# simonsobs/pixell

Measured on AMD Instinct MI355X. Metric: map2alm+alm2map round-trips/sec, higher is better.
Workload: dtype f64

## Files before the change

pixell_amd/csrc/leg_s0.hip:

```cpp
#include "legendre_dev.hpp"

namespace pxs {

#define S0_PHASE_A \
	while (k + 4 <= nk) { \
		bool act = false; \
		_Pragma("unroll") for (int s = 0; s < K; s++) act |= LEG_IS_LIVE(lam2[s], sc[s]); \
		if (__any(act)) break; \
		const double4_t q0 = LDC(coef, k), q1 = LDC(coef, k+1), q2 = LDC(coef, k+2), q3 = LDC(coef, k+3); \
		const double b0 = polar ? q0.c : q0.b, b1 = polar ? q1.c : q1.b, b2 = polar ? q2.c : q2.b, b3 = polar ? q3.c : q3.b; \
		_Pragma("unroll") for (int s = 0; s < K; s++) { \
			lam1[s] = fma(fma(q0.a, csq[s], b0), lam2[s], lam1[s]); \
			lam2[s] = fma(fma(q1.a, csq[s], b1), lam1[s], lam2[s]); \
			lam1[s] = fma(fma(q2.a, csq[s], b2), lam2[s], lam1[s]); \
			lam2[s] = fma(fma(q3.a, csq[s], b3), lam1[s], lam2[s]); \
			if (sc[s] < 0 && fabs(lam2[s]) > SC_BIG) { lam1[s] *= SC_SMALL; lam2[s] *= SC_SMALL; sc[s]++; } \
		} \
		k += 4; \
	}
#define S0_SEEDED_PHASE_A \
	if (a.seed_mode == 2) { \
		const double* sd = a.seed_d + ((long)m*a.nwave + wv)*(2*K*64); const int* si = a.seed_i + ((long)m*a.nwave + wv)*((K+1)*64); \
		k = PXS_UNIFORM_INT(si[K*64]); \
		_Pragma("unroll") for (int s = 0; s < K; s++) { lam1[s] = sd[s*64 + lane]; lam2[s] = sd[(K+s)*64 + lane]; sc[s] = si[s*64 + lane]; } \
// ... 117 lines not shown
	double t0 = 0, t1 = 0, t2 = 0, t3 = 0, u0 = 0, u1 = 0, u2 = 0, u3 = 0; \
	_Pragma("unroll") for (int s = 0; s < K; s++) { \
		t0 = fma(lam2[s], d1r[s], t0); t1 = fma(lam2[s], d1i[s], t1); t2 = fma(lam2[s], d2r[s], t2); t3 = fma(lam2[s], d2i[s], t3); \
		lam1[s] = fma(fma(c0.a, csq[s], vb0), lam2[s], lam1[s]); \
	} \
	_Pragma("unroll") for (int s = 0; s < K; s++) { \
		u0 = fma(lam1[s], d1r[s], u0); u1 = fma(lam1[s], d1i[s], u1); u2 = fma(lam1[s], d2r[s], u2); u3 = fma(lam1[s], d2i[s], u3); \
		lam2[s] = fma(fma(c1.a, csq[s], vb1), lam1[s], lam2[s]); \
	} \
	 \
	LEG_RED_PUT(kk, t0, t1, t2, t3) \
	LEG_RED_PUT(kk+1, u0, u1, u2, u3) \
	kk += 2; \
	if (kk == LEG_FSTEPS) { leg_flush(red, pout + 4*kbase, lane, LEG_FSTEPS, a.atomic); kk = 0; kbase = k+2; } }

template<int K> __global__ __launch_bounds__(64) void leg_ana_s0(const LegK a)
{
	PXS_SHARED(double, red);
	const int lane = threadIdx.x; int wv, m, bb;
	if (!leg_block(a, wv, m, bb)) return;
	const long row0 = PXS_UNIFORM_LONG(a.row[m]);
	const int nk = (a.lmax - m)/2 + 1;
	const double4_t* __restrict__ coef = a.coef + row0;
	double* __restrict__ pout = a.part + (long)bb*a.mom_bs + ((long)wv*a.rows_chunk + (row0 - a.rowbase))*4;
	const double2* __restrict__ in = a.leg + (long)bb*a.leg_bs + (long)m*a.ld;
	double csq[K], lam1[K], lam2[K], d1r[K], d1i[K], d2r[K], d2i[K];
	int sc[K];
	bool alive_any = false;
	const bool polar = leg_wave_polar(a, wv, K);
	auto load_data = [&](int s) {
		const int p = leg_pair(a, wv, K, s, lane);
		const bool valid = leg_pair_valid(a, p);
		const int rn = valid ? a.ring_n[p] : -1, rs = valid ? a.ring_s[p] : -1;
		const double x = valid ? a.cth[p] : 0.0;
		const double2 vn = rn >= 0 ? in[rn] : make_double2(0, 0);
		const double2 vs = rs >= 0 ? in[rs] : make_double2(0, 0);
		d1r[s] = vn.x + vs.x; d1i[s] = vn.y + vs.y;
		d2r[s] = (vn.x - vs.x)*x; d2i[s] = (vn.y - vs.y)*x;
	};
#pragma unroll
	for (int s = 0; s < K; s++) {
		const int p = leg_pair(a, wv, K, s, lane);
		const bool valid = leg_pair_valid(a, p);
		const double x = valid ? a.cth[p] : 0.0;
		const double sth = valid ? a.sth[p] : 0.0;
		csq[s] = polar ? -sth*sth : x*x;
// ... 16 lines not shown
		bool pend = false;
#pragma unroll
		for (int s = 0; s < K; s++) pend |= (sc[s] < 0);
		if (!__any(pend)) break;
		for (int it = 0; it < 2 && k + 1 < nk; it++, k += 2) {
			const double4_t c0 = LDC(coef, k), c1 = LDC(coef, k+1);
			S0_ANA_PAIR(c0, c1)
		}
#pragma unroll
		for (int s = 0; s < K; s++)
			if (sc[s] < 0 && fabs(lam2[s]) > SC_BIG) {
				lam1[s] *= SC_SMALL; lam2[s] *= SC_SMALL;
				if (++sc[s] == 0) load_data(s);
			}
	}
	double4_t c0 = LDC(coef, k), c1 = LDC(coef, k+1);
	while (k + 3 < nk) {
		double4_t n0 = LDC(coef, k+2), n1 = LDC(coef, k+3);
		S0_ANA_PAIR(c0, c1)
		k += 2;
		c0 = LDC(coef, k+2); c1 = LDC(coef, k+3);
		S0_ANA_PAIR(n0, n1)
		k += 2;
	}
	for (; k + 1 < nk; k += 2) {
		const double4_t n0 = LDC(coef, k+2), n1 = LDC(coef, k+3);
		S0_ANA_PAIR(c0, c1)
		c0 = n0; c1 = n1;
	}
	if (k < nk) {
		double t0 = 0, t1 = 0, t2 = 0, t3 = 0;
#pragma unroll
		for (int s = 0; s < K; s++) { t0 = fma(lam2[s], d1r[s], t0); t1 = fma(lam2[s], d1i[s], t1); t2 = fma(lam2[s], d2r[s], t2); t3 = fma(lam2[s], d2i[s], t3); }
		LEG_RED_PUT(kk, t0, t1, t2, t3)
		kk++;
	}
	if (kk > 0) leg_flush(red, pout + 4*kbase, lane, kk, a.atomic);
}


struct S0Chain {
	double csq, lam1, lam2; int sc;
	__device__ __forceinline__ double step(double ca, double cb) { const double p = lam2, nx = fma(mm_coef(ca, csq, cb), lam2, lam1); lam1 = p; lam2 = nx; return p; }
	__device__ __forceinline__ void rescale() { if (fabs(lam2) > SC_BIG) { lam1 *= SC_SMALL; lam2 *= SC_SMALL; sc++; } }
// ... 65 lines not shown
					const double val = c < 2 ? fma(x, o, v) : fma(-x, v, o);
					const int ring = valid ? (c < 2 ? a.ring_n[p] : a.ring_s[p]) : -1;
					if (ring >= 0) out[2*ring] = val;
				}
		}
	}
};
template<int NG, int W> __global__ __launch_bounds__(64*W, 4) void leg_ana_s0_mm(const LegK a) { leg_ana_mm<S0Mm, NG, W>(a); }



template<int NG> __global__ __launch_bounds__(64, 4) void leg_syn_s0_mm(const LegK a) { leg_syn_mm<S0Mm, NG>(a); }

void launch_leg_s0(bool analysis, int ng, int K, dim3 grid, hipStream_t st, const LegK& a) {
	static const bool once = leg_mm_lds_optin({leg_ana_s0_mm<2, MM_WAVES>, leg_ana_s0_mm<1, MM_WAVES>}); (void)once;
	const LegKernel k = analysis ? (ng == 2 ? leg_ana_s0_mm<2, MM_WAVES> : ng ? leg_ana_s0_mm<1, MM_WAVES> : K == 8 ? leg_ana_s0<8> : K == 2 ? leg_ana_s0<2> : leg_ana_s0<4>)
	                             : (ng == 2 ? leg_syn_s0_mm<2> : ng ? leg_syn_s0_mm<1> : K == 2 ? leg_syn_s0<2> : leg_syn_s0<4>);
	leg_launch(k, analysis, ng, grid, st, a);
}

}
```

pixell_amd/csrc/leg_spin.hip:

```cpp
#include "legendre_dev.hpp"

namespace pxs {

template<int K> struct SpinState {
	double x[K], gp1[K], gp2[K], gm1[K], gm2[K];
	int scp[K], scm[K];
};

template<int K> __device__ __forceinline__ bool spin_init(const LegK& a, int wv, int lane, int m, SpinState<K>& S, int* rn, int* rs, bool polar) {
	const int s_ = a.spin;
	bool alive_any = false;
#pragma unroll
	for (int s = 0; s < K; s++) {
		const int p = leg_pair(a, wv, K, s, lane);
		const bool valid = leg_pair_valid(a, p);
		rn[s] = valid ? a.ring_n[p] : -1; rs[s] = valid ? a.ring_s[p] : -1;
		const double cth = valid ? a.cth[p] : 0.0;
		const double sth = valid ? a.sth[p] : 0.0;
		const double shh = valid ? a.sh2[p] : 0.0;
		S.x[s] = polar ? -2.0*shh*shh : cth;
		const double t1 = a.lmax*sth + a.ofs;
		const double b = -2.0*s_*fabs(cth);
		const double c = (double)s_*s_ - t1*t1;
		const double discr = b*b - 4*c;
// ... 45 lines not shown
		j = PXS_UNIFORM_INT(si[2*K*64]); \
		_Pragma("unroll") for (int s = 0; s < K; s++) { \
			S.gp1[s] = sd[s*64 + lane]; S.gp2[s] = sd[(K+s)*64 + lane]; S.gm1[s] = sd[(2*K+s)*64 + lane]; S.gm2[s] = sd[(3*K+s)*64 + lane]; \
			S.scp[s] = si[s*64 + lane]; S.scm[s] = si[(K+s)*64 + lane]; } \
	} else { \
		SPIN_PHASE_A \
		if (a.seed_mode == 1) { \
			double* sd = a.seed_d + ((long)m*a.nwave + wv)*(4*K*64); int* si = a.seed_i + ((long)m*a.nwave + wv)*((2*K+1)*64); \
			_Pragma("unroll") for (int s = 0; s < K; s++) { \
				sd[s*64 + lane] = S.gp1[s]; sd[(K+s)*64 + lane] = S.gp2[s]; sd[(2*K+s)*64 + lane] = S.gm1[s]; sd[(3*K+s)*64 + lane] = S.gm2[s]; \
				si[s*64 + lane] = S.scp[s]; si[(K+s)*64 + lane] = S.scm[s]; } \
			if (lane == 0) si[2*K*64] = j; \
		} \
	}

#define SPIN_SYN_PAIR(f0, f1, a0, a1) { \
	{ \
		const double ca = f0.a, c1 = polar ? f0.c : f0.b, c2 = polar ? f0.d : -f0.b; \
		PXS_VCOPY(v1, c1); PXS_VCOPY(v2, c2); \
		_Pragma("unroll") for (int s = 0; s < K; s++) { \
			const double gp = S.gp2[s], gm = S.gm2[s]; \
			pnr[s] = fma(gp, a0.a, pnr[s]); pni[s] = fma(gp, a0.b, pni[s]); \
			mnr[s] = fma(gm, a0.c, mnr[s]); mni[s] = fma(gm, a0.d, mni[s]); \
			qsr[s] = fma(gm, a0.a, qsr[s]); qsi[s] = fma(gm, a0.b, qsi[s]); \
			nsr[s] = fma(gp, a0.c, nsr[s]); nsi[s] = fma(gp, a0.d, nsi[s]); \
			S.gp1[s] = fma(fma(ca, S.x[s], v1), gp, -S.gp1[s]); S.gm1[s] = fma(fma(ca, S.x[s], v2), gm, -S.gm1[s]); \
		} \
	} \
	{ \
		const double ca = f1.a, c1 = polar ? f1.c : f1.b, c2 = polar ? f1.d : -f1.b; \
		PXS_VCOPY(v1, c1); PXS_VCOPY(v2, c2); \
		_Pragma("unroll") for (int s = 0; s < K; s++) { \
			const double gp = S.gp1[s], gm = S.gm1[s]; \
			pnr[s] = fma(gp, a1.a, pnr[s]); pni[s] = fma(gp, a1.b, pni[s]); \
			mnr[s] = fma(gm, a1.c, mnr[s]); mni[s] = fma(gm, a1.d, mni[s]); \
			qsr[s] = fma(-gm, a1.a, qsr[s]); qsi[s] = fma(-gm, a1.b, qsi[s]); \
			nsr[s] = fma(-gp, a1.c, nsr[s]); nsi[s] = fma(-gp, a1.d, nsi[s]); \
			S.gp2[s] = fma(fma(ca, S.x[s], v1), gp, -S.gp2[s]); S.gm2[s] = fma(fma(ca, S.x[s], v2), gm, -S.gm2[s]); \
		} \
	} }

template<int K> __global__ __launch_bounds__(64) void leg_syn_spin(const LegK a)
{
	const int lane = threadIdx.x; int wv, m, bb;
	if (!leg_block(a, wv, m, bb)) return;
	const int l0 = max(m, a.spin);
	const int nl = a.lmax - l0 + 1;
	double2* __restrict__ outq = a.leg + (long)bb*a.leg_bs + (long)m*a.ld;
	double2* __restrict__ outu = a.leg + (long)bb*a.leg_bs + ((long)a.nm + m)*a.ld;
	SpinState<K> S; int rn[K], rs[K];
	double pnr[K], pni[K], mnr[K], mni[K], qsr[K], qsi[K], nsr[K], nsi[K];
#pragma unroll
	for (int s = 0; s < K; s++) pnr[s] = pni[s] = mnr[s] = mni[s] = qsr[s] = qsi[s] = nsr[s] = nsi[s] = 0;
	const bool polar = leg_wave_polar(a, wv, K);
	const bool alive_any = spin_init<K>(a, wv, lane, m, S, rn, rs, polar);
// ... 18 lines not shown
			}
#pragma unroll
			for (int s = 0; s < K; s++) {
				const bool was = (S.scp[s] < 0) || (S.scm[s] < 0);
				if (S.scp[s] < 0 && fabs(S.gp2[s]) > SC_BIG) { S.gp1[s] *= SC_SMALL; S.gp2[s] *= SC_SMALL; S.scp[s]++; }
				if (S.scm[s] < 0 && fabs(S.gm2[s]) > SC_BIG) { S.gm1[s] *= SC_SMALL; S.gm2[s] *= SC_SMALL; S.scm[s]++; }
				if (was && S.scp[s] == 0 && S.scm[s] == 0) pnr[s] = pni[s] = mnr[s] = mni[s] = qsr[s] = qsi[s] = nsr[s] = nsi[s] = 0;
			}
		}
#pragma unroll
		for (int s = 0; s < K; s++)
			if (S.scp[s] < 0 || S.scm[s] < 0) {
				pnr[s] = pni[s] = mnr[s] = mni[s] = qsr[s] = qsi[s] = nsr[s] = nsi[s] = 0;
				S.gp1[s] = S.gp2[s] = S.gm1[s] = S.gm2[s] = 0;
			}
		double4_t f0 = LDC(coef, j), f1 = LDC(coef, j+1), a0 = LDC(at, j), a1 = LDC(at, j+1);
		while (j + 3 < nl) {
			double4_t n0 = LDC(coef, j+2), n1 = LDC(coef, j+3), m0 = LDC(at, j+2), m1 = LDC(at, j+3);
			SPIN_SYN_PAIR(f0, f1, a0, a1)
			j += 2;
			f0 = LDC(coef, j+2); f1 = LDC(coef, j+3); a0 = LDC(at, j+2); a1 = LDC(at, j+3);
			SPIN_SYN_PAIR(n0, n1, m0, m1)
			j += 2;
		}
		for (; j + 1 < nl; j += 2) {
			const double4_t n0 = LDC(coef, j+2), n1 = LDC(coef, j+3), m0 = LDC(at, j+2), m1 = LDC(at, j+3);
			SPIN_SYN_PAIR(f0, f1, a0, a1)
			f0 = n0; f1 = n1; a0 = m0; a1 = m1;
		}
		if (j < nl) {
#pragma unroll
			for (int s = 0; s < K; s++) {
				const double gp = S.gp2[s], gm = S.gm2[s];
				pnr[s] = fma(gp, a0.a, pnr[s]); pni[s] = fma(gp, a0.b, pni[s]);
				mnr[s] = fma(gm, a0.c, mnr[s]); mni[s] = fma(gm, a0.d, mni[s]);
				qsr[s] = fma(gm, a0.a, qsr[s]); qsi[s] = fma(gm, a0.b, qsi[s]);
				nsr[s] = fma(gp, a0.c, nsr[s]); nsi[s] = fma(gp, a0.d, nsi[s]);
			}
		}
	}
#pragma unroll
	for (int s = 0; s < K; s++) {
		const int p = leg_pair(a, wv, K, s, lane);
		const bool valid = leg_pair_valid(a, p);
// ... 30 lines not shown
		_Pragma("unroll") for (int s = 0; s < K; s++) { \
			const double gp = S.gp1[s], gm = S.gm1[s]; \
			u0 = fma(gp, tpnr[s], u0); u0 = fma(-gm, tpsr[s], u0); \
			u1 = fma(gp, tpni[s], u1); u1 = fma(-gm, tpsi[s], u1); \
			u2 = fma(gm, tmnr[s], u2); u2 = fma(-gp, tmsr[s], u2); \
			u3 = fma(gm, tmni[s], u3); u3 = fma(-gp, tmsi[s], u3); \
			S.gp2[s] = fma(fma(ca, S.x[s], v1), gp, -S.gp2[s]); S.gm2[s] = fma(fma(ca, S.x[s], v2), gm, -S.gm2[s]); \
		} \
	} \
	 \
	LEG_RED_PUT(kk, t0, t1, t2, t3) \
	LEG_RED_PUT(kk+1, u0, u1, u2, u3) \
	kk += 2; \
	if (kk == LEG_FSTEPS) { leg_flush(red, pout + 4*jbase, lane, LEG_FSTEPS, a.atomic); kk = 0; jbase = j+2; } }

template<int K> __global__ __launch_bounds__(64) void leg_ana_spin(const LegK a)
{
	PXS_SHARED(double, red);
	const int lane = threadIdx.x; int wv, m, bb;
	if (!leg_block(a, wv, m, bb)) return;
	const int l0 = max(m, a.spin);
	const int nl = a.lmax - l0 + 1;
	if (nl <= 0) return;
	const long row0 = PXS_UNIFORM_LONG(a.row[m]);
	const double4_t* __restrict__ coef = a.coef + row0;
	double* __restrict__ pout = a.part + (long)bb*a.mom_bs + ((long)wv*a.rows_chunk + (row0 - a.rowbase))*4;
	const double2* __restrict__ inq = a.leg + (long)bb*a.leg_bs + (long)m*a.ld;
	const double2* __restrict__ inu = a.leg + (long)bb*a.leg_bs + ((long)a.nm + m)*a.ld;
	SpinState<K> S; int rn[K], rs[K];
	const bool polar = leg_wave_polar(a, wv, K);
	const bool alive_any = spin_init<K>(a, wv, lane, m, S, rn, rs, polar);
	if (!__any(alive_any)) return;
	const double sgn0 = ((l0 + m) & 1) ? -1.0 : 1.0;
	double tpnr[K], tpni[K], tmnr[K], tmni[K], tpsr[K], tpsi[K], tmsr[K], tmsi[K];
	auto load_data = [&](int s) {
		const int p = leg_pair(a, wv, K, s, lane);
		const bool valid = leg_pair_valid(a, p);
		const int rn_ = valid ? a.ring_n[p] : -1, rs_ = valid ? a.ring_s[p] : -1;
		double2 q = rn_ >= 0 ? inq[rn_] : make_double2(0, 0), u = rn_ >= 0 ? inu[rn_] : make_double2(0, 0);
		tpnr[s] = q.x - u.y; tpni[s] = q.y + u.x; tmnr[s] = q.x + u.y; tmni[s] = q.y - u.x;
		q = rs_ >= 0 ? inq[rs_] : make_double2(0, 0); u = rs_ >= 0 ? inu[rs_] : make_double2(0, 0);
		tpsr[s] = sgn0*(q.x - u.y); tpsi[s] = sgn0*(q.y + u.x); tmsr[s] = sgn0*(q.x + u.y); tmsi[s] = sgn0*(q.y - u.x);
	};
#pragma unroll
	for (int s = 0; s < K; s++) tpnr[s] = tpni[s] = tmnr[s] = tmni[s] = tpsr[s] = tpsi[s] = tmsr[s] = tmsi[s] = 0;
	int j = 0;
	SPIN_SEEDED_PHASE_A
	j = PXS_UNIFORM_INT(j); coef = (const double4_t*)PXS_UNIFORM_LONG((long)coef);
	PXS_COUNT(1, (long)(nl - j)*K*12 + (a.seed_mode != 2 ? (long)j*K*4 : 0L));
	if (lane == 0 && !a.atomic) a.first[wv*a.nmc + (m - a.m0)] = j + 1;
#pragma unroll
// ... 4 lines not shown
#pragma unroll
		for (int s = 0; s < K; s++) pend |= (S.scp[s] < 0) || (S.scm[s] < 0);
		if (!__any(pend)) break;
		for (int it = 0; it < 2 && j + 1 < nl; it++, j += 2) {
			const double4_t f0 = LDC(coef, j), f1 = LDC(coef, j+1);
			SPIN_ANA_PAIR(f0, f1)
		}
#pragma unroll
		for (int s = 0; s < K; s++) {
			const bool was = (S.scp[s] < 0) || (S.scm[s] < 0);
			if (S.scp[s] < 0 && fabs(S.gp2[s]) > SC_BIG) { S.gp1[s] *= SC_SMALL; S.gp2[s] *= SC_SMALL; S.scp[s]++; }
			if (S.scm[s] < 0 && fabs(S.gm2[s]) > SC_BIG) { S.gm1[s] *= SC_SMALL; S.gm2[s] *= SC_SMALL; S.scm[s]++; }
			if (was && S.scp[s] == 0 && S.scm[s] == 0) load_data(s);
		}
	}
	double4_t f0 = LDC(coef, j), f1 = LDC(coef, j+1);
	while (j + 3 < nl) {
		double4_t n0 = LDC(coef, j+2), n1 = LDC(coef, j+3);
		SPIN_ANA_PAIR(f0, f1)
		j += 2;
		f0 = LDC(coef, j+2); f1 = LDC(coef, j+3);
		SPIN_ANA_PAIR(n0, n1)
		j += 2;
	}
	for (; j + 1 < nl; j += 2) {
		const double4_t n0 = LDC(coef, j+2), n1 = LDC(coef, j+3);
		SPIN_ANA_PAIR(f0, f1)
		f0 = n0; f1 = n1;
	}
	if (j < nl) {
		double t0 = 0, t1 = 0, t2 = 0, t3 = 0;
#pragma unroll
		for (int s = 0; s < K; s++) {
			const double gp = S.gp2[s], gm = S.gm2[s];
			t0 = fma(gp, tpnr[s], t0); t0 = fma(gm, tpsr[s], t0);
			t1 = fma(gp, tpni[s], t1); t1 = fma(gm, tpsi[s], t1);
			t2 = fma(gm, tmnr[s], t2); t2 = fma(gp, tmsr[s], t2);
			t3 = fma(gm, tmni[s], t3); t3 = fma(gp, tmsi[s], t3);
		}
		LEG_RED_PUT(kk, t0, t1, t2, t3)
		kk++;
	}
	if (kk > 0) leg_flush(red, pout + 4*jbase, lane, kk, a.atomic);
}
// ... 90 lines not shown
					const int ring = valid ? (c < 2 ? a.ring_n[p] : a.ring_s[p]) : -1;
					if (ring >= 0) {
						if (c & 1) { outq[2*ring + 1] = sum; outu[2*ring] = dif; }
						else       { outq[2*ring] = sum; outu[2*ring + 1] = -dif; }
					}
				}
		}
	}
};
template<int NG, int W> __global__ __launch_bounds__(64*W, 4) void leg_ana_spin_mm(const LegK a) { leg_ana_mm<SpinMm, NG, W>(a); }

template<int NG> __global__ __launch_bounds__(64, 4) void leg_syn_spin_mm(const LegK a) { leg_syn_mm<SpinMm, NG>(a); }

void launch_leg_spin(bool analysis, int ng, int K, dim3 grid, hipStream_t st, const LegK& a) {
	static const bool once = leg_mm_lds_optin({leg_ana_spin_mm<2, MM_WAVES>, leg_ana_spin_mm<1, MM_WAVES>}); (void)once;
	const LegKernel k = analysis ? (ng == 2 ? leg_ana_spin_mm<2, MM_WAVES> : ng ? leg_ana_spin_mm<1, MM_WAVES> : K >= 4 ? leg_ana_spin<4> : K == 3 ? leg_ana_spin<3> : leg_ana_spin<2>)
	                             : (ng == 2 ? leg_syn_spin_mm<2> : ng ? leg_syn_spin_mm<1> : K == 3 ? leg_syn_spin<3> : leg_syn_spin<2>);
	leg_launch(k, analysis, ng, grid, st, a);
}

}
```

pixell_amd/csrc/legendre.hip:

```cpp
#include "legendre_dev.hpp"
#include <thread>
#include <memory>
#include <functional>
#include <string>

namespace pxs {

static constexpr int K_SYN0 = 4, K_ANA0 = 8, K_SYNS = 3, K_ANAS = 4;

__device__ __forceinline__ double2 ld_alm(const void* alm, int dtype, long idx) {
	if (dtype == PX_C64) { float2 v = ((const float2*)alm)[idx]; return make_double2(v.x, v.y); }
	return ((const double2*)alm)[idx];
}
__device__ __forceinline__ void st_alm(void* alm, int dtype, long idx, double2 v) {
	if (dtype == PX_C64) ((float2*)alm)[idx] = make_float2((float)v.x, (float)v.y);
	else ((double2*)alm)[idx] = v;
}
__device__ __forceinline__ double eps_lm(int l, int m) {
	if (l <= m) return 0.0;
	double L = l, M = m;
	return sqrt((L*L - M*M)/(4.0*L*L - 1.0));
}

struct AlmK {
// ... 495 lines not shown

static int k_small_grid(const RingSet& rs, int kdef, std::initializer_list<int> smaller, int kmid = 0) {
#ifdef PXS_HOST_SIM
	const bool off = [] { const char* e = getenv("PXS_K_SMALL_OFF"); return e && atoi(e) != 0; }();
#else
	constexpr bool off = false;
#endif
	if (off || rs.npairs <= 0) return kdef;
	if (rs.npairs <= 512) { int k = kdef; for (int c : smaller) k = std::min(k, c); return k; }
	if (kmid > 0 && rs.npairs <= 1400) return kmid;
	auto eligible = [&](int k) { const int last = leg_wave_last_pair(rs.npairs, k, 0); return last >= 0 && rs.cth[last]*rs.cth[last] > PXS_POLAR_COS2; };
	if (eligible(kdef)) return kdef;
	for (int k : smaller) if (k < kdef && eligible(k)) return k;
	return kdef;
}
enum LegForm { LEG_VALU, LEG_MM8, LEG_MM4 };
struct LegLaunch { int b0, n; LegForm form; int ng; };
static int mm_min(const char* name) { const char* e = getenv(name); const int x = e ? atoi(e) : 4; return x <= 0 ? (1 << 30) : std::max(2, x); }
static int syn_mm_min() { return mm_min("PXS_SYN_MM_MIN"); }
static int ana_mm_min() { return mm_min("PXS_ANA_MM_MIN"); }
static std::vector<LegLaunch> leg_batch_plan(int nb, int spin, bool analysis, int deriv1, bool deterministic, const std::function<bool()>& seeds_pending, int max_valu, int max_mm8) {
	const bool ordered = analysis && deterministic;
	const bool mm = nb >= (analysis ? ana_mm_min() : syn_mm_min()) && !ordered && !(analysis && spin > 0 && deriv1);
	std::vector<LegLaunch> plan;
	int b = 0;
	if (mm) {
		const int nmm = nb - (nb % 8 == 1 ? 1 : 0), r = nmm % 8, n8 = nmm - r;
		for (; b < n8; b += max_mm8) plan.push_back({b, std::min(max_mm8, n8 - b), LEG_MM8, 2});
		if (r > 4) plan.push_back({n8, r, LEG_MM8, 2}); else if (r > 0) plan.push_back({n8, r, LEG_MM4, 1});
		b = nmm;
// ... 82 lines not shown
		if (prof) prof->end(st, 1);
		if (atomic) continue;
		const long maxrow = tb.row[m0+1] - tb.row[m0];
		hipLaunchKernelGGL(reduce_partials, dim3((unsigned)((4*maxrow+255)/256), m1-m0), dim3(256), 0, st, (const double*)wk.part.p,
			mom, tb.d_row.as<long>(), (const int*)wk.first.p, m0, m1-m0, tb.row[m0], rows, a.nwave);
	}
	seeds_written(seeds, st);
}

void leg_analysis(hipStream_t st, const RingSet& rs, const LegTables& tb, LegWork& wk,
                  const double2* leg, void* alm, int alm_dtype, long alm_cstride, const uint64_t* d_mstart, long lstride,
                  int deriv1, LegProfile* prof, long ld, int nb, long alm_bstride, long leg_bstride)
{
	PXS_REQUIRE(alm_dtype == PX_C64 || alm_dtype == PX_C128, "alm must be complex64 or complex128");
	PXS_REQUIRE(nb >= 1, "leg_analysis: nb must be >= 1");
	const int K = tb.spin == 0 ? k_small_grid(rs, K_ANA0, {4, 2}, 4) : k_small_grid(rs, K_ANAS, {3, 2});
	const int nm = tb.mmax+1;
	const int mm_pairs = (tb.spin == 0 ? 64 : 32)*MM_WAVES;
	const std::vector<LegLaunch> plan = leg_batch_plan(nb, tb.spin, true, deriv1, wk.deterministic, [&] { return seeds_pending(wk, rs, tb, 1, K); },
		leg_max_batch(rs, tb, 64*K, wk.max_batch), 8*leg_max_batch(rs, tb, mm_pairs, wk.max_batch));
	print_batch_plan(true, tb.spin, nb, plan);
	const size_t nmom = (size_t)leg_mom_stride(tb);
	wk.mom.ensure(sizeof(double)*nmom*nb);
	if (!wk.deterministic) PXS_HIP(hipMemsetAsync(wk.mom.p, 0, sizeof(double)*nmom*nb, st));
	wk.pass_valu.begin(); wk.pass_mm.begin();
	for (const LegLaunch& l : plan) {
		(l.ng ? wk.pass_mm : wk.pass_valu).add(l.n);
		const double2* legl = leg + (size_t)l.b0*leg_bstride;
		double* mom = wk.mom.as<double>() + nmom*l.b0;
		if (!l.ng) { leg_analysis_valu(st, rs, tb, wk, K, legl, mom, prof, ld, l.n, leg_bstride); continue; }
		LegK a = make_legk_mm(rs, tb, wk, const_cast<double2*>(legl), ld, mm_pairs, l.n, l.ng, leg_bstride);
// ... 13 lines not shown
```

pixell_amd/csrc/legendre.hpp:

```cpp
#pragma once
#include <map>
#include <tuple>
#include "common.hpp"

namespace pxs {

struct RingSet {
	int nring = 0;
	int npairs = 0;
	std::vector<int> ring_n, ring_s;
	std::vector<double> cth, sth, sh2, ch2;
	DevBuf d_ring_n, d_ring_s, d_cth, d_sth, d_sh2, d_ch2;
	void build(const std::vector<long double>& theta);
	void upload_all();
};

struct LegTables {
	int lmax = 0, mmax = 0, spin = 0;
	std::vector<long> row;
	long nrows = 0;
	DevBuf d_row, d_coef, d_alpha;
	DevBuf d_coef2, d_coef2p;
	void build_compact();
	void build(int lmax, int mmax, int spin);
// ... 10 lines not shown
	~LegProfile();
};

struct LegWork {
	size_t part_budget = size_t(2) << 30;
	bool deterministic = false;
	DevBuf almt;
	DevBuf part;
	DevBuf mom;
	DevBuf first;
	struct Seeds { DevBuf d, i; bool ready = false, refused = false; hipEvent_t written = nullptr; hipStream_t wstream = nullptr;
	               ~Seeds() { if (written) (void)hipEventDestroy(written); } };
	std::map<std::tuple<const void*, int, int, int>, Seeds> seeds;
	size_t seed_budget = size_t(16) << 30, seed_bytes = 0;
	DevBuf count; bool count_on = false;
	int max_batch = 0;
	PassLog pass_m, pass_valu, pass_mm;
};


void leg_synthesis(hipStream_t st, const RingSet& rs, const LegTables& tb, LegWork& wk,
                   const void* alm, int alm_dtype, long alm_cstride, const uint64_t* d_mstart, long lstride,
                   double2* leg, int deriv1, LegProfile* prof = nullptr, long ld = 0, int nb = 1, long alm_bstride = 0, long leg_bstride = 0);
void leg_analysis(hipStream_t st, const RingSet& rs, const LegTables& tb, LegWork& wk,
                  const double2* leg, void* alm, int alm_dtype, long alm_cstride, const uint64_t* d_mstart, long lstride,
                  int deriv1, LegProfile* prof = nullptr, long ld = 0, int nb = 1, long alm_bstride = 0, long leg_bstride = 0);

}
```

pixell_amd/csrc/legendre_dev.hpp:

```cpp
#pragma once
#include "legendre.hpp"
#include <cmath>
#include <algorithm>
#include <initializer_list>

namespace pxs {

static constexpr double SC_BIG   = 0x1p+400;
static constexpr double SC_SMALL = 0x1p-800;
static constexpr int    SC_STEP  = 800;
static constexpr double LEG_LIVE = 0x1p-140;
#define LEG_IS_LIVE(v, sc) ((sc) == 0 && fabs(v) >= LEG_LIVE)

struct double4_t { double a, b, c, d; };
#ifdef PXS_HOST_SIM
#define LDC(p, i) ((p)[i])
#else
typedef double pxs_d4 __attribute__((ext_vector_type(4)));
__device__ __forceinline__ double4_t ldc_row(const double4_t* p, long i) {
	const __attribute__((address_space(4))) pxs_d4* c = (const __attribute__((address_space(4))) pxs_d4*)(unsigned long long)p;
	const pxs_d4 v = c[i]; double4_t r; r.a = v.x; r.b = v.y; r.c = v.z; r.d = v.w; return r;
}
#define LDC(p, i) ldc_row((p), (i))
#endif
// ... 9 lines not shown

struct coef2x2_t { double a0, b0, a1, b1; };
#ifdef PXS_HOST_SIM
#define LDC2(p, i) (coef2x2_t{(p)[i].x, (p)[i].y, (p)[(i)+1].x, (p)[(i)+1].y})
#define PXS_ROWS_DRAIN()
#define PXS_ROWS_ISSUED()
#else
typedef double pxs_d4a16 __attribute__((ext_vector_type(4), aligned(16)));
__device__ __forceinline__ coef2x2_t ldc_row2(const double2* p, long i) {
	const __attribute__((address_space(4))) pxs_d4a16* c = (const __attribute__((address_space(4))) pxs_d4a16*)(unsigned long long)(p + i);
	const pxs_d4a16 v = *c; coef2x2_t r; r.a0 = v.x; r.b0 = v.y; r.a1 = v.z; r.b1 = v.w; return r;
}
#define LDC2(p, i) ldc_row2((p), (i))
#define PXS_ROWS_DRAIN() do { __builtin_amdgcn_s_waitcnt(0xc07f); __builtin_amdgcn_sched_barrier(0); } while (0)
#define PXS_ROWS_ISSUED() __builtin_amdgcn_sched_barrier(0)
#endif

struct LegK {
	int lmax, mmax, spin, nm, npairs, nring, nwave;
	long ld;
	long nrows;
	const long* row; const double4_t* coef; const double* alpha;
	const int* ring_n; const int* ring_s; const double* cth; const double* sth; const double* sh2; const double* ch2;
	double* almt; double* part; double* mom;
	double2* leg;
	double ofs;
	int m0; long rowbase, rows_chunk;
	int nmc, xcd;
	int* first;
	int atomic;
// ... 59 lines not shown
__device__ __forceinline__ int leg_pair(const LegK& a, int wv, int K, int s, int lane) { return leg_pair_of(a.npairs, a.nwave, K, wv, s, lane); }
__device__ __forceinline__ bool leg_pair_valid(const LegK& a, int p) { return (unsigned)p < (unsigned)a.npairs; }
__device__ __forceinline__ bool leg_wave_polar(const LegK& a, int wv, int K) { return mm_wave_polar(a, leg_wave_last_pair(a.npairs, K, wv) + 1); }

#ifdef PXS_HOST_SIM
#define PXS_VCOPY(dst, src) double dst = (src)
#else
#define PXS_VCOPY(dst, src) double dst; asm("v_mov_b64 %0, %1" : "=v"(dst) : "s"(src))
#endif

#ifdef PXS_HOST_SIM
#define PXS_FRESH_INT(x) (x)
#else
__device__ __forceinline__ int pxs_fresh_int(int x) { asm("" : "+v"(x)); return x; }
#define PXS_FRESH_INT(x) pxs_fresh_int(x)
#endif


#ifdef PXS_HOST_SIM
#define PXS_UNIFORM_INT(x) (x)
#define PXS_UNIFORM_LONG(x) (x)
#else
#define PXS_UNIFORM_INT(x) __builtin_amdgcn_readfirstlane(x)
#define PXS_UNIFORM_LONG(x) ((long)(((unsigned long)(unsigned)__builtin_amdgcn_readfirstlane((int)((unsigned long)(x) >> 32)) << 32) | (unsigned long)(unsigned)__builtin_amdgcn_readfirstlane((int)(unsigned long)(x))))
#endif
__device__ __forceinline__ int leg_pair_u(const LegK& a, int wv, int K, int s, int lane) { return PXS_UNIFORM_INT(leg_pair(a, wv, K, s, 0)) + lane; }


#ifdef PXS_HOST_SIM
#define PXS_WAVE_LDS_SYNC() pxsim::wave_sync()
// ... 340 lines not shown
```

pixell_amd/csrc/sht.hip:

```cpp
#include "sht_plan.hpp"
#include <cmath>
#include <algorithm>

static const char* const ROUTE_NAMES[] = {"direct", "via-cc", "via-cc-unfused", "via-cc-unfused-h", "ring-weights", "cc-weights", "chain", "unfused"};

Route::Scratch Route::scratch(const pxs_plan* p, int nb) const {
	Scratch s; const size_t nct = (size_t)nb*nc, nm = (size_t)p->mmax + 1, c16 = sizeof(double2);
	s.leg = c16*nct*nm*ld_leg_alloc; s.leg2 = c16*nct*nm*ld_leg2; s.h = c16*nct*nr_h*ld_h;
	if (to_map) s.almt = sizeof(double)*4*(tb->nrows + 4)*nb; else s.mom = sizeof(double)*4*std::max<long>(tb->nrows, 1)*nb;
	if (theta_fused && !line) FftChain::theta_scratch(theta, form->tp, (int)nm, (int)nct, s.c1, s.c2);
	if (reserve_chain) p->chain->ring_scratch(p->nring, (int)nct, !to_map, s.r1, p->mmax);
	return s;
}

namespace {

void plan_common(pxs_plan* p, int lmax, int mmax, const uint64_t* mstart, int64_t lstride, int device) {
	PXS_REQUIRE(lmax >= 0 && mmax >= 0 && mmax <= lmax, "need 0 <= mmax <= lmax");
	PXS_REQUIRE(mstart != nullptr, "mstart is required");
	PXS_HIP(hipSetDevice(device));
	p->device = device; p->lmax = lmax; p->mmax = mmax; p->lstride = lstride;
	std::vector<uint64_t> ms(mstart, mstart+mmax+1);
	p->d_mstart = upload(ms);
	p->fc = &fft_context(device);
// ... 217 lines not shown
		return 0;
	}
	if (std::string(name) == "analysis") {
		PXS_REQUIRE(value >= 0 && value <= 2, "pxs_plan_option: analysis takes 0 (interpolant), 1 (weights) or 2 (ducc0)");
		p->ana_weights = (int)value;
	} else if (std::string(name) == "deterministic") {
		PXS_REQUIRE(value == 0 || value == 1, "pxs_plan_option: deterministic takes 0 or 1");
		p->wk.deterministic = value != 0;
	} else if (std::string(name) == "build_tables") {
		PXS_REQUIRE(value >= 0 && value <= p->lmax + 1, "pxs_plan_option: build_tables takes a spin");
		PXS_HIP(hipSetDevice(p->device));
		(void)p->table((int)value);
	} else if (std::string(name) == "leg_max_batch") {
		PXS_REQUIRE(value >= 0 && value <= (1 << 20), "pxs_plan_option: leg_max_batch takes 0 (no bound) or a number of maps");
		p->wk.max_batch = (int)value;
	} else throw Error(PXS_ERR_ARG, std::string("pxs_plan_option: unknown option '") + name + "'");
	PXS_CATCH
}

static const AnaForm& ana_form(const pxs_plan* p) { return p->ana_weights != 0 && p->ana_fine.M > 0 ? p->ana_fine : p->ana_interp; }

static void run_theta(pxs_plan* p, hipStream_t st, const Route& r, int nct, int spin, const double2* wring) {
	const ThetaTables& t = p->th; const AnaForm& f = *r.form;
	const bool to_h = r.theta == TH_FROM_CC || r.theta == TH_TO_CC_ADJ, mid = r.theta == TH_TO_CC || r.theta == TH_TO_CC_ADJ;
	ThetaCall c;
	c.tp = &f.tp; c.nc = nct; c.nm = p->mmax + 1; c.spin = spin; c.lmax = p->lmax; c.mir_c = t.mir_c;
	c.map = (to_h ? p->hbuf : p->leg).as<double2>(); c.ldmap = to_h ? r.ld_h : r.ld_leg; c.nr = to_h ? r.nr_h : r.nr_th;
	c.cc = p->leg2.as<double2>(); c.ldcc = r.ld_leg2; c.ncc = t.ncc;
	c.ph = (r.theta == TH_FROM_CC ? t.ph_up : t.ph_shift).as<double2>();
	if (mid) c.sigma = f.sigma.as<double2>();
// ... 43 lines not shown
		const PassLog* l = nullptr;
		if (seam == "fft") { int dev = p ? p->device : 0; if (!p) PXS_HIP(hipGetDevice(&dev)); l = &fft_context(dev).pass_lines; }
		else {
			PXS_REQUIRE(p && !p->pts, "pxs_plan_query: the passes of this seam belong to a grid or ring plan");
			if (seam == "batch") l = &p->pass_batch; else if (seam == "resample") l = &p->pass_resample;
			else if (seam == "leg_m") l = &p->wk.pass_m; else if (seam == "leg_valu") l = &p->wk.pass_valu; else if (seam == "leg_mm") l = &p->wk.pass_mm;
			else if ((seam == "theta" || seam == "ring") && p->chain) l = seam == "theta" ? &p->chain->pass_theta : &p->chain->pass_ring;
		}
		if (!l) throw Error(PXS_ERR_ARG, std::string("pxs_plan_query: unknown name '") + name + "'");
		*value = which == 0 ? l->n : which == 1 ? l->first : which == 2 ? l->prev : l->last;
		return 0;
	}
	PXS_REQUIRE(p, "pxs_plan_query: null argument");
	if (p->pts) *value = points_query(p->pts, n);
	else if (n == "analysis_form") { const Route r = analysis_route_now(p); *value = (r.kind == R_RING_WEIGHTS || r.kind == R_CC_WEIGHTS) ? 1 : (r.form->fine ? 2 : 0); }
	else if (n == "ncc_circle") *value = p->th.ncc > 0 ? p->th.Ncc : 0;
	else if (n == "ducc_ncc_circle") *value = FftChain::ducc_ncc(p->lmax);
	else if (n == "theta_line") *value = analysis_route_now(p).line ? 1 : 0;
	else if (n == "chain_stages" || n == "chain_static") {
		int64_t k = 0;
		for (const ChainShape& c : chain_shapes(p)) {
			if (getenv("PXS_CHAIN_VERBOSE")) fprintf(stderr, "[pxsht] plan stage %d: na=%d nb=%d T=%d static %d\n", c.sid, c.na, c.nb, c.T, c.is_static ? 1 : 0);
			k += (n == "chain_stages" || c.is_static) ? 1 : 0;
		}
		*value = k;
	}
	else if (n == "chain_static_table") *value = p->chain ? p->chain->static_check(0) : 0;
	else throw Error(PXS_ERR_ARG, std::string("pxs_plan_query: unknown name '") + name + "'");
	PXS_CATCH
}
// ... 277 lines not shown
```

Before: 3.674.

## Software-pipeline coefficient row loads in VALU Legendre kernels and add K=6 spin analysis

```diff
diff --git a/pixell_amd/csrc/leg_s0.hip b/pixell_amd/csrc/leg_s0.hip
--- a/pixell_amd/csrc/leg_s0.hip
+++ b/pixell_amd/csrc/leg_s0.hip
@@ -155,6 +155,26 @@
 	kk += 2; \
 	if (kk == LEG_FSTEPS) { leg_flush(red, pout + 4*kbase, lane, LEG_FSTEPS, a.atomic); kk = 0; kbase = k+2; } }
 
+#define S0_ANA_STEP_C(ca, cb, LA, LB, T0, T1, T2, T3) { \
+	PXS_VCOPY(vb, cb); \
+	_Pragma("unroll") for (int s = 0; s < K; s++) { \
+		T0 = fma(LA[s], d1r[s], T0); T1 = fma(LA[s], d1i[s], T1); T2 = fma(LA[s], d2r[s], T2); T3 = fma(LA[s], d2i[s], T3); \
+		LB[s] = fma(fma(ca, csq[s], vb), LA[s], LB[s]); \
+	} }
+#define S0_ANA_PAIR_D(ca0, cb0, ca1, cb1, kfirst, NEXT) { \
+	double t0 = 0, t1 = 0, t2 = 0, t3 = 0, u0 = 0, u1 = 0, u2 = 0, u3 = 0; \
+	S0_ANA_STEP_C(ca0, cb0, lam2, lam1, t0, t1, t2, t3) \
+	_Pragma("unroll") for (int s = 0; s < K; s++) PXS_DONE(lam1[s]); \
+	PXS_DONE(t0); PXS_DONE(t1); PXS_DONE(t2); PXS_DONE(t3); \
+	PXS_ROWS_DRAIN(); \
+	if (kk == LEG_FSTEPS) { leg_flush(red, pout + 4*kbase, lane, LEG_FSTEPS, a.atomic); kk = 0; kbase = (kfirst); } \
+	NEXT; \
+	PXS_ROWS_ISSUED(); \
+	S0_ANA_STEP_C(ca1, cb1, lam1, lam2, u0, u1, u2, u3) \
+	LEG_RED_PUT(kk, t0, t1, t2, t3) \
+	LEG_RED_PUT(kk+1, u0, u1, u2, u3) \
+	kk += 2; }
+
 template<int K> __global__ __launch_bounds__(64) void leg_ana_s0(const LegK a)
 {
 	PXS_SHARED(double, red);
@@ -170,7 +190,7 @@
 	bool alive_any = false;
 	const bool polar = leg_wave_polar(a, wv, K);
 	auto load_data = [&](int s) {
-		const int p = leg_pair(a, wv, K, s, lane);
+		const int p = leg_pair(a, wv, K, s, PXS_LATE_INT(lane));
 		const bool valid = leg_pair_valid(a, p);
 		const int rn = valid ? a.ring_n[p] : -1, rs = valid ? a.ring_s[p] : -1;
 		const double x = valid ? a.cth[p] : 0.0;
@@ -217,20 +237,21 @@
 				if (++sc[s] == 0) load_data(s);
 			}
 	}
-	double4_t c0 = LDC(coef, k), c1 = LDC(coef, k+1);
+	const double2* __restrict__ cf = (const double2*)PXS_UNIFORM_LONG((long)((polar ? a.coef2p : a.coef2) + row0));
+	coef2x2_t n = LDC2(cf, k), f = LDC2(cf, k+1);
+	PXS_ROWS_DRAIN();
+	n.a1 = n.a0; n.b1 = n.b0;
 	while (k + 3 < nk) {
-		double4_t n0 = LDC(coef, k+2), n1 = LDC(coef, k+3);
-		S0_ANA_PAIR(c0, c1)
+		S0_ANA_PAIR_D(n.a1, n.b1, f.a0, f.b0, k, n = LDC2(cf, k+3))
+		S0_ANA_PAIR_D(f.a1, f.b1, n.a0, n.b0, k+2, f = LDC2(cf, k+5))
+		k += 4;
+	}
+	if (k + 1 < nk) {
+		S0_ANA_PAIR_D(n.a1, n.b1, f.a0, f.b0, k, (void)0)
 		k += 2;
-		c0 = LDC(coef, k+2); c1 = LDC(coef, k+3);
-		S0_ANA_PAIR(n0, n1)
-		k += 2;
-	}
-	for (; k + 1 < nk; k += 2) {
-		const double4_t n0 = LDC(coef, k+2), n1 = LDC(coef, k+3);
-		S0_ANA_PAIR(c0, c1)
-		c0 = n0; c1 = n1;
-	}
+	}
+	PXS_ROWS_DRAIN();
+	if (kk == LEG_FSTEPS) { leg_flush(red, pout + 4*kbase, lane, LEG_FSTEPS, a.atomic); kk = 0; kbase = k; }
 	if (k < nk) {
 		double t0 = 0, t1 = 0, t2 = 0, t3 = 0;
 #pragma unroll
@@ -326,8 +347,9 @@
 
 void launch_leg_s0(bool analysis, int ng, int K, dim3 grid, hipStream_t st, const LegK& a) {
 	static const bool once = leg_mm_lds_optin({leg_ana_s0_mm<2, MM_WAVES>, leg_ana_s0_mm<1, MM_WAVES>}); (void)once;
-	const LegKernel k = analysis ? (ng == 2 ? leg_ana_s0_mm<2, MM_WAVES> : ng ? leg_ana_s0_mm<1, MM_WAVES> : K == 8 ? leg_ana_s0<8> : K == 2 ? leg_ana_s0<2> : leg_ana_s0<4>)
-	                             : (ng == 2 ? leg_syn_s0_mm<2> : ng ? leg_syn_s0_mm<1> : K == 2 ? leg_syn_s0<2> : leg_syn_s0<4>);
+	const LegKernel k = analysis ? (ng == 2 ? leg_ana_s0_mm<2, MM_WAVES> : ng ? leg_ana_s0_mm<1, MM_WAVES> : K == 8 ? leg_ana_s0<8> : K == 4 ? leg_ana_s0<4> : K == 2 ? leg_ana_s0<2> : nullptr)
+	                             : (ng == 2 ? leg_syn_s0_mm<2> : ng ? leg_syn_s0_mm<1> : K == 4 ? leg_syn_s0<4> : K == 2 ? leg_syn_s0<2> : nullptr);
+	PXS_REQUIRE(k != nullptr, "internal: no spin-0 Legendre kernel compiled for this number of ring pairs per lane");
 	leg_launch(k, analysis, ng, grid, st, a);
 }
 
diff --git a/pixell_amd/csrc/leg_spin.hip b/pixell_amd/csrc/leg_spin.hip
--- a/pixell_amd/csrc/leg_spin.hip
+++ b/pixell_amd/csrc/leg_spin.hip
@@ -83,9 +83,15 @@
 		} \
 	}
 
-#define SPIN_SYN_PAIR(f0, f1, a0, a1) { \
+struct spin_rows_t { double4_t r0, r1; };
+__device__ __forceinline__ spin_rows_t spin_rows(const double4_t* coef, long i) { spin_rows_t r; r.r0 = LDC(coef, i); r.r1 = LDC(coef, i+1); return r; }
+#define SPIN_ROW0(r) r.r0.a, polar ? r.r0.c : r.r0.b, polar ? r.r0.d : -r.r0.b
+#define SPIN_ROW1(r) r.r1.a, polar ? r.r1.c : r.r1.b, polar ? r.r1.d : -r.r1.b
+
+#define SPIN_SYN_PAIR(f0, f1, a0, a1) SPIN_SYN_PAIR_C(f0.a, polar ? f0.c : f0.b, polar ? f0.d : -f0.b, f1.a, polar ? f1.c : f1.b, polar ? f1.d : -f1.b, a0, a1)
+#define SPIN_SYN_PAIR_C(ca0, c10, c20, ca1, c11, c21, a0, a1) { \
 	{ \
-		const double ca = f0.a, c1 = polar ? f0.c : f0.b, c2 = polar ? f0.d : -f0.b; \
+		const double ca = ca0, c1 = c10, c2 = c20; \
 		PXS_VCOPY(v1, c1); PXS_VCOPY(v2, c2); \
 		_Pragma("unroll") for (int s = 0; s < K; s++) { \
 			const double gp = S.gp2[s], gm = S.gm2[s]; \
@@ -97,7 +103,7 @@
 		} \
 	} \
 	{ \
-		const double ca = f1.a, c1 = polar ? f1.c : f1.b, c2 = polar ? f1.d : -f1.b; \
+		const double ca = ca1, c1 = c11, c2 = c21; \
 		PXS_VCOPY(v1, c1); PXS_VCOPY(v2, c2); \
 		_Pragma("unroll") for (int s = 0; s < K; s++) { \
 			const double gp = S.gp1[s], gm = S.gm1[s]; \
@@ -108,6 +114,29 @@
 			S.gp2[s] = fma(fma(ca, S.x[s], v1), gp, -S.gp2[s]); S.gm2[s] = fma(fma(ca, S.x[s], v2), gm, -S.gm2[s]); \
 		} \
 	} }
+
+#define SPIN_SYN_PAIR_R(s0, s1, a0, a1) SPIN_SYN_PAIR_C(s0, s1, a0, a1)
+#define SPIN_SYN_PHASE_C { \
+	spin_rows_t f = spin_rows(coef, j); a0 = LDC(at, j); a1 = LDC(at, j+1); \
+	while (j + 3 < nl) { \
+		PXS_ROWS_DRAIN(); \
+		spin_rows_t n = spin_rows(coef, j+2); double4_t m0 = LDC(at, j+2), m1 = LDC(at, j+3); \
+		PXS_ROWS_ISSUED(); \
+		SPIN_SYN_PAIR_R(SPIN_ROW0(f), SPIN_ROW1(f), a0, a1) \
+		PXS_ROWS_DRAIN(); \
+		f = spin_rows(coef, j+4); a0 = LDC(at, j+4); a1 = LDC(at, j+5); \
+		PXS_ROWS_ISSUED(); \
+		SPIN_SYN_PAIR_R(SPIN_ROW0(n), SPIN_ROW1(n), m0, m1) \
+		j += 4; \
+	} \
+	for (; j + 1 < nl; j += 2) { \
+		PXS_ROWS_DRAIN(); \
+		const spin_rows_t n = spin_rows(coef, j+2); const double4_t m0 = LDC(at, j+2), m1 = LDC(at, j+3); \
+		PXS_ROWS_ISSUED(); \
+		SPIN_SYN_PAIR_R(SPIN_ROW0(f), SPIN_ROW1(f), a0, a1) \
+		f = n; a0 = m0; a1 = m1; \
+	} \
+	PXS_ROWS_DRAIN(); }
 
 template<int K> __global__ __launch_bounds__(64) void leg_syn_spin(const LegK a)
 {
@@ -156,20 +185,8 @@
 				pnr[s] = pni[s] = mnr[s] = mni[s] = qsr[s] = qsi[s] = nsr[s] = nsi[s] = 0;
 				S.gp1[s] = S.gp2[s] = S.gm1[s] = S.gm2[s] = 0;
 			}
-		double4_t f0 = LDC(coef, j), f1 = LDC(coef, j+1), a0 = LDC(at, j), a1 = LDC(at, j+1);
-		while (j + 3 < nl) {
-			double4_t n0 = LDC(coef, j+2), n1 = LDC(coef, j+3), m0 = LDC(at, j+2), m1 = LDC(at, j+3);
-			SPIN_SYN_PAIR(f0, f1, a0, a1)
-			j += 2;
-			f0 = LDC(coef, j+2); f1 = LDC(coef, j+3); a0 = LDC(at, j+2); a1 = LDC(at, j+3);
-			SPIN_SYN_PAIR(n0, n1, m0, m1)
-			j += 2;
-		}
-		for (; j + 1 < nl; j += 2) {
-			const double4_t n0 = LDC(coef, j+2), n1 = LDC(coef, j+3), m0 = LDC(at, j+2), m1 = LDC(at, j+3);
-			SPIN_SYN_PAIR(f0, f1, a0, a1)
-			f0 = n0; f1 = n1; a0 = m0; a1 = m1;
-		}
+		double4_t a0, a1;
+		SPIN_SYN_PHASE_C
 		if (j < nl) {
 #pragma unroll
 			for (int s = 0; s < K; s++) {
@@ -230,7 +247,55 @@
 	kk += 2; \
 	if (kk == LEG_FSTEPS) { leg_flush(red, pout + 4*jbase, lane, LEG_FSTEPS, a.atomic); kk = 0; jbase = j+2; } }
 
-template<int K> __global__ __launch_bounds__(64) void leg_ana_spin(const LegK a)
+#define SPIN_ANA_STEP0_C(ca, c1, c2) { \
+	PXS_VCOPY(v1, c1); PXS_VCOPY(v2, c2); \
+	_Pragma("unroll") for (int s = 0; s < K; s++) { \
+		const double gp = S.gp2[s], gm = S.gm2[s]; \
+		t0 = fma(gp, tpnr[s], t0); t0 = fma(gm, tpsr[s], t0); \
+		t1 = fma(gp, tpni[s], t1); t1 = fma(gm, tpsi[s], t1); \
+		t2 = fma(gm, tmnr[s], t2); t2 = fma(gp, tmsr[s], t2); \
+		t3 = fma(gm, tmni[s], t3); t3 = fma(gp, tmsi[s], t3); \
+		S.gp1[s] = fma(fma(ca, S.x[s], v1), gp, -S.gp1[s]); S.gm1[s] = fma(fma(ca, S.x[s], v2), gm, -S.gm1[s]); \
+	} }
+#define SPIN_ANA_STEP1_C(ca, c1, c2) { \
+	PXS_VCOPY(v1, c1); PXS_VCOPY(v2, c2); \
+	_Pragma("unroll") for (int s = 0; s < K; s++) { \
+		const double gp = S.gp1[s], gm = S.gm1[s]; \
+		u0 = fma(gp, tpnr[s], u0); u0 = fma(-gm, tpsr[s], u0); \
+		u1 = fma(gp, tpni[s], u1); u1 = fma(-gm, tpsi[s], u1); \
+		u2 = fma(gm, tmnr[s], u2); u2 = fma(-gp, tmsr[s], u2); \
+		u3 = fma(gm, tmni[s], u3); u3 = fma(-gp, tmsi[s], u3); \
+		S.gp2[s] = fma(fma(ca, S.x[s], v1), gp, -S.gp2[s]); S.gm2[s] = fma(fma(ca, S.x[s], v2), gm, -S.gm2[s]); \
+	} }
+#define SPIN_ANA_PAIR_D(ca0, c10, c20, ca1, c11, c21, jfirst, NEXT) { \
+	double t0 = 0, t1 = 0, t2 = 0, t3 = 0, u0 = 0, u1 = 0, u2 = 0, u3 = 0; \
+	SPIN_ANA_STEP0_C(ca0, c10, c20) \
+	_Pragma("unroll") for (int s = 0; s < K; s++) { PXS_DONE(S.gp1[s]); PXS_DONE(S.gm1[s]); } \
+	PXS_DONE(t0); PXS_DONE(t1); PXS_DONE(t2); PXS_DONE(t3); \
+	PXS_ROWS_DRAIN(); \
+	if (kk == LEG_FSTEPS) { leg_flush(red, pout + 4*jbase, lane, LEG_FSTEPS, a.atomic); kk = 0; jbase = (jfirst); } \
+	NEXT; \
+	PXS_ROWS_ISSUED(); \
+	SPIN_ANA_STEP1_C(ca1, c11, c21) \
+	LEG_RED_PUT(kk, t0, t1, t2, t3) \
+	LEG_RED_PUT(kk+1, u0, u1, u2, u3) \
+	kk += 2; }
+#define SPIN_ANA_PHASE_C { \
+	spin_rows_t n = spin_rows(coef, j), f = spin_rows(coef, j+1); \
+	PXS_ROWS_DRAIN(); \
+	n.r1 = n.r0; \
+	while (j + 3 < nl) {       \
+		SPIN_ANA_PAIR_R(SPIN_ROW1(n), SPIN_ROW0(f), j, n = spin_rows(coef, j+3)) \
+		SPIN_ANA_PAIR_R(SPIN_ROW1(f), SPIN_ROW0(n), j+2, f = spin_rows(coef, j+5)) \
+		j += 4; \
+	} \
+	if (j + 1 < nl) { \
+		SPIN_ANA_PAIR_R(SPIN_ROW1(n), SPIN_ROW0(f), j, (void)0) \
+		j += 2; \
+	} }
+#define SPIN_ANA_PAIR_R(s0, s1, jfirst, NEXT) SPIN_ANA_PAIR_D(s0, s1, jfirst, NEXT)
+
+template<int K> __global__ __launch_bounds__(64, (K == 2 ? 5 : 1)) void leg_ana_spin(const LegK a)
 {
 	PXS_SHARED(double, red);
 	const int lane = threadIdx.x; int wv, m, bb;
@@ -250,7 +315,7 @@
 	const double sgn0 = ((l0 + m) & 1) ? -1.0 : 1.0;
 	double tpnr[K], tpni[K], tmnr[K], tmni[K], tpsr[K], tpsi[K], tmsr[K], tmsi[K];
 	auto load_data = [&](int s) {
-		const int p = leg_pair(a, wv, K, s, lane);
+		const int p = leg_pair(a, wv, K, s, PXS_LATE_INT(lane));
 		const bool valid = leg_pair_valid(a, p);
 		const int rn_ = valid ? a.ring_n[p] : -1, rs_ = valid ? a.ring_s[p] : -1;
 		double2 q = rn_ >= 0 ? inq[rn_] : make_double2(0, 0), u = rn_ >= 0 ? inu[rn_] : make_double2(0, 0);
@@ -285,20 +350,9 @@
 			if (was && S.scp[s] == 0 && S.scm[s] == 0) load_data(s);
 		}
 	}
-	double4_t f0 = LDC(coef, j), f1 = LDC(coef, j+1);
-	while (j + 3 < nl) {
-		double4_t n0 = LDC(coef, j+2), n1 = LDC(coef, j+3);
-		SPIN_ANA_PAIR(f0, f1)
-		j += 2;
-		f0 = LDC(coef, j+2); f1 = LDC(coef, j+3);
-		SPIN_ANA_PAIR(n0, n1)
-		j += 2;
-	}
-	for (; j + 1 < nl; j += 2) {
-		const double4_t n0 = LDC(coef, j+2), n1 = LDC(coef, j+3);
-		SPIN_ANA_PAIR(f0, f1)
-		f0 = n0; f1 = n1;
-	}
+	SPIN_ANA_PHASE_C
+	PXS_ROWS_DRAIN();
+	if (kk == LEG_FSTEPS) { leg_flush(red, pout + 4*jbase, lane, LEG_FSTEPS, a.atomic); kk = 0; jbase = j; }
 	if (j < nl) {
 		double t0 = 0, t1 = 0, t2 = 0, t3 = 0;
 #pragma unroll
@@ -419,8 +473,9 @@
 
 void launch_leg_spin(bool analysis, int ng, int K, dim3 grid, hipStream_t st, const LegK& a) {
 	static const bool once = leg_mm_lds_optin({leg_ana_spin_mm<2, MM_WAVES>, leg_ana_spin_mm<1, MM_WAVES>}); (void)once;
-	const LegKernel k = analysis ? (ng == 2 ? leg_ana_spin_mm<2, MM_WAVES> : ng ? leg_ana_spin_mm<1, MM_WAVES> : K >= 4 ? leg_ana_spin<4> : K == 3 ? leg_ana_spin<3> : leg_ana_spin<2>)
-	                             : (ng == 2 ? leg_syn_spin_mm<2> : ng ? leg_syn_spin_mm<1> : K == 3 ? leg_syn_spin<3> : leg_syn_spin<2>);
+	const LegKernel k = analysis ? (ng == 2 ? leg_ana_spin_mm<2, MM_WAVES> : ng ? leg_ana_spin_mm<1, MM_WAVES> : K == 6 ? leg_ana_spin<6> : K == 4 ? leg_ana_spin<4> : K == 3 ? leg_ana_spin<3> : K == 2 ? leg_ana_spin<2> : nullptr)
+	                             : (ng == 2 ? leg_syn_spin_mm<2> : ng ? leg_syn_spin_mm<1> : K == 3 ? leg_syn_spin<3> : K == 2 ? leg_syn_spin<2> : nullptr);
+	PXS_REQUIRE(k != nullptr, "internal: no spin-s Legendre kernel compiled for this number of ring pairs per lane");
 	leg_launch(k, analysis, ng, grid, st, a);
 }
 
diff --git a/pixell_amd/csrc/legendre.hip b/pixell_amd/csrc/legendre.hip
--- a/pixell_amd/csrc/legendre.hip
+++ b/pixell_amd/csrc/legendre.hip
@@ -533,6 +533,12 @@
 	for (int k : smaller) if (k < kdef && eligible(k)) return k;
 	return kdef;
 }
+static constexpr int K_ANAS_BIG = 6, LEG_BIG_MIN_WAVES = 8;
+static int leg_ana_k(const RingSet& rs, int spin) {
+	if (spin == 0) return k_small_grid(rs, K_ANA0, {4, 2}, 4);
+	const int k = k_small_grid(rs, K_ANAS, {3, 2});
+	return (k == K_ANAS && (rs.npairs + 64*K_ANAS - 1)/(64*K_ANAS) >= LEG_BIG_MIN_WAVES) ? K_ANAS_BIG : k;
+}
 enum LegForm { LEG_VALU, LEG_MM8, LEG_MM4 };
 struct LegLaunch { int b0, n; LegForm form; int ng; };
 static int mm_min(const char* name) { const char* e = getenv(name); const int x = e ? atoi(e) : 4; return x <= 0 ? (1 << 30) : std::max(2, x); }
@@ -645,7 +651,8 @@
 {
 	PXS_REQUIRE(alm_dtype == PX_C64 || alm_dtype == PX_C128, "alm must be complex64 or complex128");
 	PXS_REQUIRE(nb >= 1, "leg_analysis: nb must be >= 1");
-	const int K = tb.spin == 0 ? k_small_grid(rs, K_ANA0, {4, 2}, 4) : k_small_grid(rs, K_ANAS, {3, 2});
+	const int K = wk.ana_k > 0 ? wk.ana_k : leg_ana_k(rs, tb.spin);
+	wk.last_ana_k = K;
 	const int nm = tb.mmax+1;
 	const int mm_pairs = (tb.spin == 0 ? 64 : 32)*MM_WAVES;
 	const std::vector<LegLaunch> plan = leg_batch_plan(nb, tb.spin, true, deriv1, wk.deterministic, [&] { return seeds_pending(wk, rs, tb, 1, K); },
diff --git a/pixell_amd/csrc/legendre.hpp b/pixell_amd/csrc/legendre.hpp
--- a/pixell_amd/csrc/legendre.hpp
+++ b/pixell_amd/csrc/legendre.hpp
@@ -48,6 +48,8 @@
 	std::map<std::tuple<const void*, int, int, int>, Seeds> seeds;
 	size_t seed_budget = size_t(16) << 30, seed_bytes = 0;
 	DevBuf count; bool count_on = false;
+	int ana_k = 0;
+	int last_ana_k = 0;
 	int max_batch = 0;
 	PassLog pass_m, pass_valu, pass_mm;
 };
diff --git a/pixell_amd/csrc/legendre_dev.hpp b/pixell_amd/csrc/legendre_dev.hpp
--- a/pixell_amd/csrc/legendre_dev.hpp
+++ b/pixell_amd/csrc/legendre_dev.hpp
@@ -47,6 +47,11 @@
 #define LDC2(p, i) ldc_row2((p), (i))
 #define PXS_ROWS_DRAIN() do { __builtin_amdgcn_s_waitcnt(0xc07f); __builtin_amdgcn_sched_barrier(0); } while (0)
 #define PXS_ROWS_ISSUED() __builtin_amdgcn_sched_barrier(0)
+#endif
+#ifdef PXS_HOST_SIM
+#define PXS_DONE(x)
+#else
+#define PXS_DONE(x) asm volatile("" : "+v"(x))
 #endif
 
 struct LegK {
@@ -136,6 +141,12 @@
 #else
 __device__ __forceinline__ int pxs_fresh_int(int x) { asm("" : "+v"(x)); return x; }
 #define PXS_FRESH_INT(x) pxs_fresh_int(x)
+#endif
+#ifdef PXS_HOST_SIM
+#define PXS_LATE_INT(x) (x)
+#else
+__device__ __forceinline__ int pxs_late_int(int x) { asm volatile("" : "+v"(x)); return x; }
+#define PXS_LATE_INT(x) pxs_late_int(x)
 #endif
 
 
diff --git a/pixell_amd/csrc/sht.hip b/pixell_amd/csrc/sht.hip
--- a/pixell_amd/csrc/sht.hip
+++ b/pixell_amd/csrc/sht.hip
@@ -255,6 +255,9 @@
 	} else if (std::string(name) == "leg_max_batch") {
 		PXS_REQUIRE(value >= 0 && value <= (1 << 20), "pxs_plan_option: leg_max_batch takes 0 (no bound) or a number of maps");
 		p->wk.max_batch = (int)value;
+	} else if (std::string(name) == "leg_ana_k") {
+		PXS_REQUIRE(value >= 0 && value <= 64, "pxs_plan_option: leg_ana_k takes 0 (the host's rule) or a number of ring pairs per lane");
+		p->wk.ana_k = (int)value;
 	} else throw Error(PXS_ERR_ARG, std::string("pxs_plan_option: unknown option '") + name + "'");
 	PXS_CATCH
 }
@@ -328,6 +331,7 @@
 	PXS_REQUIRE(p, "pxs_plan_query: null argument");
 	if (p->pts) *value = points_query(p->pts, n);
 	else if (n == "analysis_form") { const Route r = analysis_route_now(p); *value = (r.kind == R_RING_WEIGHTS || r.kind == R_CC_WEIGHTS) ? 1 : (r.form->fine ? 2 : 0); }
+	else if (n == "leg_ana_k") *value = p->wk.last_ana_k;
 	else if (n == "ncc_circle") *value = p->th.ncc > 0 ? p->th.Ncc : 0;
 	else if (n == "ducc_ncc_circle") *value = FftChain::ducc_ncc(p->lmax);
 	else if (n == "theta_line") *value = analysis_route_now(p).line ? 1 : 0;
```

Result: faster. 3.742, median of 6 (+1.8%).
